# JuliaSmoothOptimizers/Krylov.jl

Hardware: NVIDIA H100
Metric: CG iterations/s (higher is better)
Workload: dtype f64

## Files before the change

krylov.jl_b200/csrc/blas1.cu:

```cuda
#include <mutex>
#include <set>
#include <utility>

#include "kb_internal.h"

#include <chrono>

namespace kb {

void ensure_dyn_smem(const void* func, int bytes) {
  static std::mutex mu;
  static std::set<std::pair<const void*, int>> done;
  int dev = 0;
  KB_CUDA(cudaGetDevice(&dev));
  std::lock_guard<std::mutex> lk(mu);
  if (done.count({func, dev})) return;
  KB_CUDA(cudaFuncSetAttribute(func, cudaFuncAttributeMaxDynamicSharedMemorySize, bytes));
  done.insert({func, dev});
}

double now_seconds() {
  using namespace std::chrono;
  return duration_cast<duration<double>>(steady_clock::now().time_since_epoch()).count();
}
// ... 265 lines not shown
  const long long code = (long long)s;
  user_exit = (code % 1024) > 0;
  overtimed = (code / 1024) > 0;
}

void dist_check_alive(Ctx& c) {
  if (!c.dcomm) return;
  int err = 0;
  KB_CUDA(cudaMemcpyAsync(&err, &c.dcomm->error, sizeof(int), cudaMemcpyDeviceToHost, c.stream));
  c.sync();
  if (err) throw std::runtime_error("cross-GPU reduction timed out: a peer rank stopped participating; the communicator of this "
                                    "workspace is dead (free the workspace on every rank and create it again)");
}

template <class T>
__global__ void __launch_bounds__(kBlock) cg_prologue_kernel(int n, const T* __restrict__ b, T* __restrict__ x, T* __restrict__ r,
                                                             T* __restrict__ p, T* part, unsigned* ticket, T* out, DistComm* dc) {
  __shared__ T sm[32];
  T acc = T(0);
  const int stride = gridDim.x * blockDim.x;
  for (int i = blockIdx.x * blockDim.x + threadIdx.x; i < n; i += stride) {
    const T v = b[i];
    x[i] = T(0); r[i] = v; p[i] = v;
    acc += v * v;
  }
  T mine[1] = {block_sum(acc, sm)}, tot[1];
  if (grid_sum_last<T, 1>(mine, part, ticket, sm, tot) && threadIdx.x == 0) out[0] = dist_reduce(dc, tot[0]);
}
template <class T> T k_cg_prologue(Ctx& c, int n, const T* b, T* x, T* r, T* p) {
  const int grid = n > 0 ? stream_grid(n, 4, 4) : 1;
  cg_prologue_kernel<T><<<grid, kBlock, 0, c.stream>>>(n, b, x, r, p, (T*)c.partials, c.tickets, slot_ptr<T>(c, 0), c.dcomm);
  KB_CUDA(cudaGetLastError());
  c.launches++;
  return read_slot<T>(c, 0);
}

#define INST(T)                                                                        \
  template T k_dot<T>(Ctx&, int, const T*, const T*);                                  \
  template T k_cg_prologue<T>(Ctx&, int, const T*, T*, T*, T*);                        \
  template T k_nrm2<T>(Ctx&, int, const T*);                                           \
  template void k_dot2<T>(Ctx&, int, const T*, const T*, const T*, const T*, T*, T*);  \
  template void k_dot_dev<T>(Ctx&, int, const T*, const T*, int);                      \
  template void k_axpy<T>(Ctx&, int, T, const T*, T*);                                 \
  template void k_axpby<T>(Ctx&, int, T, const T*, T, T*);                             \
  template void k_scal<T>(Ctx&, int, T, T*);                                           \
  template void k_copy<T>(Ctx&, int, T*, const T*);                                    \
  template void k_scalcopy<T>(Ctx&, int, T*, T, const T*);                             \
  template void k_divcopy<T>(Ctx&, int, T*, const T*, T);                              \
  template void k_fill<T>(Ctx&, int, T*, T);                                           \
  template void k_diagmul<T>(Ctx&, int, T*, const T*, const T*, bool);                 \
  template void k_blockdiag_mul<T>(Ctx&, int, int, const T*, const T*, T*);            \
  template void k_blockdiag_invert<T>(Ctx&, int, int, const T*, T*, int*);
INST(double)
INST(float)
// ... 4 lines not shown
```

krylov.jl_b200/csrc/cg_fused.cu:

```cuda
#include "solver_common.h"
#include "spmv_tiles.cuh"

namespace kb {

constexpr int kHist = 64;

template <class T>
struct CgState {
  T gamma, pAp, alpha, beta, pNorm2, rNorm, eps_tol, pad0;
  int iter, itmax, done, linesearch;
  int solved, tired, zero_curvature, inconsistent;
  int npc, not_spd, comm_error, pad2;
  T hist[kHist];
};

static_assert(sizeof(CgState<double>) % 8 == 0 && sizeof(CgState<float>) % 8 == 0, "CgState is copied as 8-byte words");

template <class T>
struct CgPeers {
  HaloMap halo;
  const T* r[kMaxRanks];
  const T* p_old[kMaxRanks];
  const T* mdiag;
  const T* r_halo;
  const T* p_halo_old;
  PushPlan<T> push_p;
};

template <class T>
// ... 335 lines not shown

template <class T>
__device__ __forceinline__ void cg_stage_halo(HaloMap halo, const CgPeerTab<T>* tab, T* r, T* p_old, int pb, int G, int tid, int nthreads) {
  const int nh = halo.nhalo, nloc = halo.nloc;
  const int per = (nh + G - 1) / G;
  const int h0 = (int)blockIdx.x * per, h1 = min(nh, h0 + per);
  for (int h = h0 + tid; h < h1; h += nthreads) {
    const int rk = __ldg(&halo.src_rank[h]), off = __ldg(&halo.src_off[h]);
    const T rv = ld_sys(tab->r[rk] + off);
    const T pv = ld_sys(tab->p[pb][rk] + off);
    __stcg(&r[nloc + h], rv);
    __stcg(&p_old[nloc + h], pv);
  }
}

template <class T, int MODE, class PhaseA>
__device__ __forceinline__ int cg_persist_iterations(int n, const CgPersistArgs<T>& a, CgState<T>* st, T* part, GridBar* gb,
                                                     DistComm* dc, T* sm, unsigned* sflag, CgScal<T>& sc, PhaseA phase_a) {
  const int G = gridDim.x, tid = threadIdx.x, lane = tid & 31;
  int passes = 0;
  for (int k = 0; k < a.max_iters; k++) {
    const int iter = sc.iter;
    const T beta = sc.beta, alpha_prev = sc.alpha;
    T* p_old = (iter & 1) ? a.P1 : a.P0;
    T* p_new = (iter & 1) ? a.P0 : a.P1;
    const bool timing = a.timed && blockIdx.x == 0 && tid == 0;
    unsigned long long t0 = 0, t1 = 0;
    if (timing) t0 = globaltimer_ns();
    const T dacc = phase_a(k, iter, beta, alpha_prev, p_old, p_new);
    passes = k + 1;
    bool ok = grid_reduce_barrier<T>(gb, dacc, part, sm, sflag, st, &sc, [&](T tot) {
      if (MODE == kDist) {
        tot = (T)dist_allreduce_sum_warp<T>(dc, (double)tot);
        if (*(volatile int*)&dc->error) { if (lane == 0) { st->comm_error = 1; st->done = 1; } return; }
      }
// ... 14 lines not shown
    }
    ok = grid_reduce_barrier<T>(gb, acc, part, sm, sflag, st, &sc, [&](T tot) {
      if (MODE == kDist) {
        tot = (T)dist_allreduce_sum_warp<T>(dc, (double)tot);
        if (*(volatile int*)&dc->error) { if (lane == 0) { st->comm_error = 1; st->done = 1; } return; }
      }
      if (lane == 0) {
        cg_k2_finalize(st, tot);
        if (MODE == kDist) gb->halo_ready = 0u;
      }
    });
    if (timing) {
      const unsigned long long t2 = globaltimer_ns();
      gb->ns_a += t1 - t0; gb->ns_b += t2 - t1; gb->timed_iters += 1;
    }
    if (!ok || sc.done) break;
  }
  return passes;
}

template <class T, int MODE, int MINB>
__global__ void __launch_bounds__(kTileThreads, MINB) cg_persist(Csr<T> A, CgPersistArgs<T> a, CgState<T>* st, T* part,
                                                                GridBar* gb, DistComm* dc) {
  extern __shared__ __align__(128) unsigned char smem[];
  __shared__ T sm[32];
  __shared__ unsigned sflag[2];
  __shared__ CgScal<T> sc;
  volatile CgState<T>* vst = st;
  if (vst->done) { cg_report_to_host<T>(a, st); return; }
  if (threadIdx.x == 0) cg_load_scal<T>(st, &sc);
  TilePipe<T> P;
// ... 177 lines not shown
    std::vector<int> fl(nt), ord;
    KB_CUDA(cudaMemcpyAsync(fl.data(), ws.dist.tile_order, sizeof(int) * nt, cudaMemcpyDeviceToHost, c.stream));
    c.sync();
    ord.reserve(nt);
    for (int t = 0; t < nt; t++) if (!fl[t]) ord.push_back(t);
    ws.dist.tile_order_interior = (int)ord.size();
    for (int t = 0; t < nt; t++) if (fl[t]) ord.push_back((int)((unsigned)t | 0x80000000u));
    KB_CUDA(cudaMemcpyAsync(ws.dist.tile_order, ord.data(), sizeof(int) * nt, cudaMemcpyHostToDevice, c.stream));
    c.sync();
  }
  ws.dist.tile_order_for = (const void*)A.rowptr;
  ws.dist.tile_order_n = nt;
}

template <class T>
CgFusedPlan<T> cg_fused_plan(const Workspace<T>& ws, const LinOp<T>& A, const LinOp<T>& M, const SolveOpts& o) {
  CgFusedPlan<T> pl;
  const bool dist = ws.dist.world > 1;
  const bool jac = M.kind == LinOp<T>::DIAG && !o.ldiv, bjac = M.kind == LinOp<T>::BDIAG && !o.ldiv;
  if (!o.fused || A.kind != LinOp<T>::CSR || o.radius != 0 || !(M.is_identity() || jac || bjac) || (dist && !M.is_identity()))
    return pl;
  const Csr<T>& C = *A.csr;
  const int n = ws.n;
  pl.single_step = (o.callback != nullptr) || (o.timemax < 1e300) || o.verbose > 0;
  const char* exu = getenv("KB200_XUP");
  pl.xup = !pl.single_step && !(exu && atoi(exu) == 0);
  pl.persist = C.tma_ok && pl.xup && o.persist != 0;
  if (bjac && !pl.persist) return pl;
  pl.fused = true;
  pl.A = &C;
  pl.mdiag = jac ? M.diag : nullptr;
  pl.mblocks = bjac ? M.blocks : nullptr;
  pl.mbs = bjac ? M.bs : 0;
  pl.batch = pl.single_step ? 1 : (o.batch > 0 ? std::min(o.batch, kHist / 2) : 32);
  if (pl.persist) {
    if (bjac) pl.kp = cg_persist<T, kBlockJac, 2>;
    else if (C.ctas_per_sm >= 3) pl.kp = dist ? cg_persist<T, kDist, 3> : (jac ? cg_persist<T, kJacobi, 3> : cg_persist<T, kPlain, 3>);
    else pl.kp = dist ? cg_persist<T, kDist, 2> : (jac ? cg_persist<T, kJacobi, 2> : cg_persist<T, kPlain, 2>);
    ensure_dyn_smem((const void*)pl.kp, 220 * 1024);
    int occ = 0;
    KB_CUDA(cudaOccupancyMaxActiveBlocksPerMultiprocessor(&occ, pl.kp, kTileThreads, C.smem_bytes));
    if (occ < 1) throw std::runtime_error("cg_persist does not fit on an SM with the planned shared-memory ring");
    pl.pgrid = std::min(std::min(occ, C.ctas_per_sm) * sm_count(), std::max(1, C.ntiles));
    const CsrDict<T>* dict = A.dict;
    if (dict && dict->npairs > 0 && dict->n == n && !dist && !bjac) {
      const typename CgFusedPlan<T>::KdFn kd =
          C.ctas_per_sm >= 3 ? (jac ? cg_persist_dict<T, kJacobi, 3> : cg_persist_dict<T, kPlain, 3>)
                             : (jac ? cg_persist_dict<T, kJacobi, 2> : cg_persist_dict<T, kPlain, 2>);
      int occd = 0;
      KB_CUDA(cudaOccupancyMaxActiveBlocksPerMultiprocessor(&occd, kd, kTileThreads, 0));
      if (occd * sm_count() >= pl.pgrid) { pl.kd = kd; pl.dict = dict; }
    }
    return pl;
  }
  const bool xup = pl.xup;
  if (C.tma_ok) {
    if (dist) pl.k1 = xup ? cg_k1_tma<T, kDist, 3, true> : cg_k1_tma<T, kDist, 3, false>;
    else if (jac) pl.k1 = xup ? cg_k1_tma<T, kJacobi, 3, true> : cg_k1_tma<T, kJacobi, 3, false>;
    else if (C.ctas_per_sm >= 4) pl.k1 = xup ? cg_k1_tma<T, kPlain, 4, true> : cg_k1_tma<T, kPlain, 4, false>;
    else if (C.ctas_per_sm == 3) pl.k1 = xup ? cg_k1_tma<T, kPlain, 3, true> : cg_k1_tma<T, kPlain, 3, false>;
    else pl.k1 = xup ? cg_k1_tma<T, kPlain, 1, true> : cg_k1_tma<T, kPlain, 1, false>;
    ensure_dyn_smem((const void*)pl.k1, 220 * 1024);
    int occ = 0;
    KB_CUDA(cudaOccupancyMaxActiveBlocksPerMultiprocessor(&occ, pl.k1, kTileThreads, C.smem_bytes));
    if (occ < 1) throw std::runtime_error("cg_k1_tma does not fit on an SM with the planned shared-memory ring");
    pl.k1_grid = std::min(std::min(occ, C.ctas_per_sm) * sm_count(), std::max(1, C.ntiles));
    pl.k1_block = kTileThreads;
    pl.k1_smem = C.smem_bytes;
  } else {
    if (dist) pl.k1 = xup ? cg_k1_rows<T, kDist, true> : cg_k1_rows<T, kDist, false>;
    else if (jac) pl.k1 = xup ? cg_k1_rows<T, kJacobi, true> : cg_k1_rows<T, kJacobi, false>;
    else pl.k1 = xup ? cg_k1_rows<T, kPlain, true> : cg_k1_rows<T, kPlain, false>;
    pl.k1_grid = stream_grid(n, 1, 8);
    pl.k1_block = kBlock;
    pl.k1_smem = 0;
  }
  if (dist) pl.k2 = xup ? cg_k2<T, kDist, false> : cg_k2<T, kDist, true>;
  else if (jac) pl.k2 = xup ? cg_k2<T, kJacobi, false> : cg_k2<T, kJacobi, true>;
  else pl.k2 = xup ? cg_k2<T, kPlain, false> : cg_k2<T, kPlain, true>;
  pl.k2_grid = stream_grid(n, 4, 8);
  return pl;
}

template <class T>
CgFusedExit cg_fused_loop(Workspace<T>& ws, const CgFusedPlan<T>& pl, const SolveOpts& o, T gamma0, T eps_tol, int itmax,
                          double start_time) {
  Ctx& c = ws.ctx;
  const int n = ws.n;
  typedef CgState<T> St;
  const bool dist = ws.dist.world > 1;
  const Csr<T>& A = *pl.A;
  cg_fused_prepare<T>(ws);
  St* dst = (St*)ws.fused_state;
  St* hst = (St*)ws.fused_host;
  auto hslot = [&](int i) -> St* { return (St*)((char*)hst + (size_t)i * kOffGridBar); };

  St init;
  memset(&init, 0, sizeof(init));
  init.gamma = gamma0; init.pNorm2 = gamma0; init.beta = T(0); init.eps_tol = eps_tol;
  init.rNorm = sqrt(gamma0); init.itmax = itmax; init.linesearch = o.linesearch ? 1 : 0;
  *hslot(0) = init;
  KB_CUDA(cudaMemcpyAsync(dst, hslot(0), sizeof(St), cudaMemcpyHostToDevice, c.stream));
  KB_CUDA(cudaMemsetAsync((char*)ws.fused_state + kOffGridBar, 0, sizeof(GridBar), c.stream));

  const bool persist = pl.persist, single_step = pl.single_step;
  const int batch = pl.batch;
  T* P[2] = {ws.p, ws.p2};
  T* part = (T*)c.partials;
  CgPeers<T> peersP[2];
  memset(peersP, 0, sizeof(peersP));
  const T* md = pl.mdiag;
  peersP[0].mdiag = md; peersP[1].mdiag = md;
  PushPlan<T> push_r;
  memset(&push_r, 0, sizeof(push_r));
  if (dist) {
    for (int b = 0; b < 2; b++) {
      peersP[b].halo = ws.dist.halo;
      const bool wantB = (b == 1) != ws.dist.swapped;
      for (int k = 0; k < ws.dist.world; k++) {
        peersP[b].r[k] = ws.dist.r_peer[k];
        peersP[b].p_old[k] = wantB ? ws.dist.bufB_peer[k] : ws.dist.bufA_peer[k];
// ... 33 lines not shown
        for (int k = 0; k < ws.dist.world; k++) {
          htab->r[k] = ws.dist.r_peer[k];
          htab->p[b][k] = wantB ? ws.dist.bufB_peer[k] : ws.dist.bufA_peer[k];
        }
      }
      CgPeerTab<T>* dtab = (CgPeerTab<T>*)((char*)ws.fused_state + kOffPeerTab);
      KB_CUDA(cudaMemcpyAsync(dtab, htab, sizeof(*htab), cudaMemcpyHostToDevice, c.stream));
      pa.halo = ws.dist.halo;
      pa.tab = dtab;
      pa.tile_order = ws.dist.tile_order;
      pa.n_interior = ws.dist.tile_order_interior;
    }
  }

  cudaEvent_t* ev = ws.fused_ev;
  int enq = 0;
  constexpr int kTimedFirst = 8, kTimedCount = 32;
  std::vector<cudaEvent_t> tev;
  if (o.time_kernels) {
    tev.resize(3 * kTimedCount);
    for (auto& e : tev) KB_CUDA(cudaEventCreate(&e));
  }
  unsigned long long* hseq = (unsigned long long*)((char*)ws.fused_host + kOffHostSeq);
  unsigned long long expect[2] = {0, 0};
  auto wait_report = [&](int slot) {
    long spins = 0;
    while (__atomic_load_n(&hseq[slot], __ATOMIC_ACQUIRE) != expect[slot]) {
      if ((++spins & 1023) == 0) {
        const cudaError_t q = cudaStreamQuery(c.stream);
        if (q != cudaSuccess && q != cudaErrorNotReady) throw CudaError(std::string("persistent CG kernel failed: ") + cudaGetErrorString(q));
        if (q == cudaSuccess && __atomic_load_n(&hseq[slot], __ATOMIC_ACQUIRE) != expect[slot])
// ... 16 lines not shown
        CsrDict<T> Dcopy = *pl.dict;
        void* args[] = {(void*)&Dcopy, (void*)&pa, (void*)&dst, (void*)&partp, (void*)&gbar};
        KB_CUDA(cudaLaunchCooperativeKernel((const void*)pl.kd, dim3(pl.pgrid), dim3(kTileThreads), args, 0, c.stream));
      } else {
        void* args[] = {(void*)&Acopy, (void*)&pa, (void*)&dst, (void*)&partp, (void*)&gbar, (void*)&dcm};
        KB_CUDA(cudaLaunchCooperativeKernel((const void*)pl.kp, dim3(pl.pgrid), dim3(kTileThreads), args, A.smem_bytes, c.stream));
      }
      c.launches += 1;
      enq += batch;
      return;
    }
    for (int b = 0; b < batch; b++, enq++) {
      T* p_old = P[enq & 1];
      T* p_new = P[(enq + 1) & 1];
      const CgPeers<T>& pe = peersP[enq & 1];
      const int ti = enq - kTimedFirst;
      const bool timed = o.time_kernels && ti >= 0 && ti < kTimedCount;
      if (timed) KB_CUDA(cudaEventRecord(tev[3 * ti], c.stream));
      DistComm* dcm = dist ? c.dcomm : nullptr;
      pl.k1<<<pl.k1_grid, pl.k1_block, pl.k1_smem, c.stream>>>(A, ws.r, p_old, p_new, ws.Ap, dst, part, c.tickets + 2, dcm, pe, ws.x);
      if (timed) KB_CUDA(cudaEventRecord(tev[3 * ti + 1], c.stream));
      pl.k2<<<pl.k2_grid, kBlock, 0, c.stream>>>(n, ws.x, ws.r, p_new, ws.Ap, dst, part, c.tickets + 3, dcm, md, push_r);
      if (timed) KB_CUDA(cudaEventRecord(tev[3 * ti + 2], c.stream));
      c.launches += 2;
    }
    KB_CUDA(cudaGetLastError());
    KB_CUDA(cudaMemcpyAsync(hslot(slot), dst, sizeof(St), cudaMemcpyDeviceToHost, c.stream));
    KB_CUDA(cudaEventRecord(ev[slot], c.stream));
  };

  int cur = 0, seen = 0;
  St last;
  bool user_exit = false, overtimed = false;
  enqueue(0);
  for (;;) {
    if (!single_step) enqueue(cur ^ 1);
    if (persist) wait_report(cur);
    else KB_CUDA(cudaEventSynchronize(ev[cur]));
    last = *hslot(cur);
    for (int k = seen + 1; k <= last.iter; k++) {
      if (o.history) ws.stats.residuals.push_back((double)last.hist[k % kHist]);
    }
    seen = last.iter;
    if (last.done) break;
    if (single_step) {
      if (o.verbose > 0 && (last.iter % o.verbose == 0))
        fprintf(stdout, "%5d  %7.1e  %8.1e  %8.1e\n", last.iter, (double)last.rNorm, (double)last.pAp, (double)last.alpha);
      if (o.callback) {
        ws.stats.niter = last.iter;
        user_exit = o.callback(&ws, o.callback_user) != 0;
      }
      overtimed = (now_seconds() - start_time) > o.timemax;
      agree_exit(ws, o, user_exit, overtimed);
      if (user_exit || overtimed) break;
      enqueue(cur);
    } else {
      cur ^= 1;
    }
  }
  c.sync();
  if (o.time_kernels && persist) {
    GridBar hb;
    KB_CUDA(cudaMemcpy(&hb, gbar, sizeof(hb), cudaMemcpyDeviceToHost));
    ws.timed_pairs = (int)hb.timed_iters;
    ws.k1_ms = hb.timed_iters ? 1e-6 * (double)hb.ns_a / hb.timed_iters : 0;
    ws.k2_ms = hb.timed_iters ? 1e-6 * (double)hb.ns_b / hb.timed_iters : 0;
    for (auto& e : tev) cudaEventDestroy(e);
  } else if (o.time_kernels) {
    const int pairs = std::min(kTimedCount, std::max(0, std::min(enq, last.iter) - kTimedFirst));
    double s1 = 0, s2 = 0;
    for (int i = 0; i < pairs; i++) {
      float a = 0, b = 0;
      cudaEventElapsedTime(&a, tev[3 * i], tev[3 * i + 1]);
      cudaEventElapsedTime(&b, tev[3 * i + 1], tev[3 * i + 2]);
      s1 += a; s2 += b;
    }
    ws.timed_pairs = pairs;
    ws.k1_ms = pairs ? s1 / pairs : 0;
    ws.k2_ms = pairs ? s2 / pairs : 0;
    for (auto& e : tev) cudaEventDestroy(e);
  }
  if (last.comm_error) throw std::runtime_error("cross-GPU all-reduce timed out: a peer rank is not participating");
  if (last.not_spd) throw std::runtime_error("The linear operator `A` or the preconditioner `M` is not symmetric positive definite.");

  const int iter = last.iter;
  const bool k1_exit = last.zero_curvature || last.npc;
  T* pcur = k1_exit ? P[(iter + 1) & 1] : P[iter & 1];
  if (pcur != ws.p) { T* tmp = ws.p; ws.p = ws.p2; ws.p2 = tmp; ws.dist.swapped = !ws.dist.swapped; }
  if (pl.xup && !k1_exit && iter > 0) k_axpy<T>(c, n, last.alpha, ws.p, ws.x);
  if (last.npc) {
    if (iter == 0) k_copy<T>(c, n, ws.x, ws.p);
    k_copy<T>(c, n, ws.npc_dir, ws.p);
    ws.stats.npcCount = 1;
    ws.stats.indefinite = true;
  }
  return CgFusedExit{iter, last.solved != 0, last.tired != 0, last.zero_curvature != 0, last.inconsistent != 0, user_exit, overtimed};
}

#define INST(T)                                                                                              \
  template CgFusedPlan<T> cg_fused_plan<T>(const Workspace<T>&, const LinOp<T>&, const LinOp<T>&, const SolveOpts&); \
  template void fused_block_alloc<T>(Workspace<T>&);                                                         \
  template void cg_fused_prepare<T>(Workspace<T>&);                                                          \
  template void cg_dist_push_r<T>(Workspace<T>&);                                                            \
  template CgFusedExit cg_fused_loop<T>(Workspace<T>&, const CgFusedPlan<T>&, const SolveOpts&, T, T, int, double);
INST(double)
INST(float)
#undef INST

}
```

krylov.jl_b200/csrc/kb_internal.h:

```cpp
#pragma once
#include <cuda_runtime.h>
#include <cstddef>
#include <cstdint>
#include <string>
#include <vector>

#include "common.cuh"
#include "dist.cuh"

namespace kb {

struct Ctx {
  int device = 0;
  cudaStream_t stream = nullptr;
  bool own_stream = false;
  void* partials = nullptr;
  unsigned* tickets = nullptr;
  void* dscal = nullptr;
  void* hscal = nullptr;
  long long launches = 0;
  DistComm* dcomm = nullptr;
  DistExchange* dex = nullptr;

  void init(int dev);
  void destroy();
  void sync() { KB_CUDA(cudaStreamSynchronize(stream)); }
};

template <class T> T* dev_alloc(size_t n);
void dev_free(void* p);

template <class T> T    k_dot(Ctx& c, int n, const T* x, const T* y);
template <class T> T    k_nrm2(Ctx& c, int n, const T* x);
template <class T> T    k_cg_prologue(Ctx& c, int n, const T* b, T* x, T* r, T* p);
template <class T> void k_dot2(Ctx& c, int n, const T* a, const T* b, const T* u, const T* v, T* r1, T* r2);
template <class T> void k_dot_dev(Ctx& c, int n, const T* x, const T* y, int slot);
template <class T> void k_axpy(Ctx& c, int n, T s, const T* x, T* y);
template <class T> void k_axpby(Ctx& c, int n, T s, const T* x, T t, T* y);
template <class T> void k_scal(Ctx& c, int n, T s, T* x);
template <class T> void k_copy(Ctx& c, int n, T* y, const T* x);
template <class T> void k_scalcopy(Ctx& c, int n, T* y, T s, const T* x);
template <class T> void k_divcopy(Ctx& c, int n, T* y, const T* x, T s);
template <class T> void k_fill(Ctx& c, int n, T* x, T v);
template <class T> void k_diagmul(Ctx& c, int n, T* y, const T* d, const T* x, bool ldiv);
template <class T> void k_blockdiag_mul(Ctx& c, int n, int bs, const T* blocks, const T* x, T* y);
template <class T> void k_blockdiag_invert(Ctx& c, int n, int bs, const T* blocks, T* inv, int* singular);
double k_dist_sum(Ctx& c, double v);
void dist_agree_on_exit(Ctx& c, bool& user_exit, bool& overtimed);
void dist_check_alive(Ctx& c);
// ... 225 lines not shown
  T *d1 = nullptr, *d2 = nullptr;
  T *Ar = nullptr, *Mr = nullptr;
  std::vector<T*> V;
  std::vector<T*> Z;
  std::vector<T> c, sgiv, zg, R;
  std::vector<T> err_vec;
  int memory = 20, window = 5;
  int inner_iter = 0;
  const T* mdiag_fused = nullptr;
  double k1_ms = 0, k2_ms = 0;
  int timed_pairs = 0;
  void* fused_state = nullptr;
  void* fused_host = nullptr;
  cudaEvent_t fused_ev[2] = {nullptr, nullptr};
  unsigned long long fused_seq = 0;
  T* bbuf = nullptr;
  T* cbuf = nullptr;
  struct Dist {
    int rank = 0, world = 1;
    HaloMap halo{0, 0, nullptr, nullptr};
    void* mailbox = nullptr;
    T* bufA_peer[kMaxRanks] = {};
    T* bufB_peer[kMaxRanks] = {};
    T* r_peer[kMaxRanks] = {};
    std::vector<void*> opened;
    bool swapped = false;
    T* halo_buf = nullptr;
    T* halo_buf_peer[kMaxRanks] = {};
    int nhalo_peer[kMaxRanks] = {};
    void* dummy[3] = {nullptr, nullptr, nullptr};
// ... 37 lines not shown
template <class T> void craig_solve(Workspace<T>& ws, const LinOp<T>& A, const LinOp<T>& At, const T* b, const LinOp<T>& M,
                                    const LinOp<T>& N, const SolveOpts& o);
template <class T> void craigmr_solve(Workspace<T>& ws, const LinOp<T>& A, const LinOp<T>& At, const T* b, const LinOp<T>& M,
                                      const LinOp<T>& N, const SolveOpts& o);
template <class T> void lnlq_solve(Workspace<T>& ws, const LinOp<T>& A, const LinOp<T>& At, const T* b, const LinOp<T>& M,
                                   const LinOp<T>& N, const SolveOpts& o);
template <class T> void cgne_solve(Workspace<T>& ws, const LinOp<T>& A, const LinOp<T>& At, const T* b, const LinOp<T>& N,
                                   const SolveOpts& o);
template <class T> void crmr_solve(Workspace<T>& ws, const LinOp<T>& A, const LinOp<T>& At, const T* b, const LinOp<T>& N,
                                   const SolveOpts& o);
template <class T> void cgls_solve(Workspace<T>& ws, const LinOp<T>& A, const LinOp<T>& At, const T* b, const LinOp<T>& M,
                                   const SolveOpts& o);
template <class T> void crls_solve(Workspace<T>& ws, const LinOp<T>& A, const LinOp<T>& At, const T* b, const LinOp<T>& M,
                                   const SolveOpts& o);

template <class T> struct CgState;
template <class T> struct CgPeers;
template <class T> struct CgPersistArgs;
struct GridBar;
template <class T>
struct CgFusedPlan {
  typedef void (*K1Fn)(Csr<T>, const T*, const T*, T*, T*, CgState<T>*, T*, unsigned*, DistComm*, CgPeers<T>, T*);
  typedef void (*K2Fn)(int, T*, T*, const T*, const T*, CgState<T>*, T*, unsigned*, DistComm*, const T*, PushPlan<T>);
  typedef void (*KpFn)(Csr<T>, CgPersistArgs<T>, CgState<T>*, T*, GridBar*, DistComm*);
  typedef void (*KdFn)(CsrDict<T>, CgPersistArgs<T>, CgState<T>*, T*, GridBar*);
  bool fused = false;
  bool persist = false;
  bool single_step = false;
  bool xup = false;
  int batch = 1;
  const Csr<T>* A = nullptr;
  const T* mdiag = nullptr;
  const T* mblocks = nullptr;
  int mbs = 0;
  K1Fn k1 = nullptr;
  K2Fn k2 = nullptr;
  int k1_grid = 0, k1_block = 0, k2_grid = 0;
  size_t k1_smem = 0;
  KpFn kp = nullptr;
  KdFn kd = nullptr;
  const CsrDict<T>* dict = nullptr;
  int pgrid = 0;
};
struct CgFusedExit { int iter; bool solved, tired, zero_curvature, inconsistent, user_exit, overtimed; };
template <class T> CgFusedPlan<T> cg_fused_plan(const Workspace<T>& ws, const LinOp<T>& A, const LinOp<T>& M, const SolveOpts& o);
template <class T> CgFusedExit cg_fused_loop(Workspace<T>& ws, const CgFusedPlan<T>& plan, const SolveOpts& o, T gamma0, T eps_tol,
                                             int itmax, double start_time);
template <class T> void cg_dist_push_r(Workspace<T>& ws);
template <class T> void cg_fused_prepare(Workspace<T>& ws);
template <class T> void fused_block_alloc(Workspace<T>& ws);
constexpr size_t kFusedBlockBytes = 4096;

template <class T> void bicgstab_fused_iteration(Workspace<T>& ws, const Csr<T>& A, const T* cvec, bool first, T rho_in, T* alpha,
                                                 T* omega, T* next_rho, T* rNorm);
template <class T> void minres_fused_lanczos(Workspace<T>& ws, const Csr<T>& A, int iter, T lambda, T beta, T oldbeta, T cs, T sn,
                                             T deltabar, T eps_rot, T* w, T* alpha, T* beta2);
template <class T> T minres_fused_update(Workspace<T>& ws, T* w, T gamma, T phi);
template <class T> void gmres_fused_arnoldi(Workspace<T>& ws, const Csr<T>& A, int k, T* h_out, T* Hbis, const T* xin = nullptr);
template <class T> void fused_multi_axpy(Workspace<T>& ws, T* xr, int k, const T* y, T* const* vecs);
template <class T> void fused_orth_chain(Workspace<T>& ws, const Csr<T>& A, const T* xin, T* q, const T* const* vecs, int cnt, T* h_out, T* Hbis);
template <class T> void trunc_fused_direction(Workspace<T>& ws, T* pp, int cnt, T* const* pvecs, const T* coefs, const T* z, T h0, T step);
template <class T> T cgs_fused_sigma(Workspace<T>& ws, const Csr<T>& A, const T* cvec);
// ... 63 lines not shown
```

krylov.jl_b200/csrc/solvers.cu:

```cuda
#include <algorithm>
#include <cmath>
#include <cstring>
#include <limits>

#include "solver_common.h"

namespace kb {

template <class T> Workspace<T>* ws_create(SolverKind kind, int m, int n, int memory, int window, int device) {
  const double t0 = now_seconds();
  const SolverInfo* info = solver_info(kind);
  if (m != n && !(info && info->rect)) throw std::runtime_error("System must be square");
  Workspace<T>* ws = new Workspace<T>();
  try {
    ws->kind = kind; ws->m = m; ws->n = n;
    ws->ctx.init(device);
    fused_block_alloc<T>(*ws);
    auto A = [&]() { return dev_alloc<T>((size_t)n); };
    ws->x = A();
    switch (kind) {
      case S_CG: ws->r = A(); ws->p = A(); ws->Ap = A(); cg_fused_prepare<T>(*ws); break;
      case S_BICGSTAB: ws->r = A(); ws->p = A(); ws->v = A(); ws->s = A(); ws->qd = A(); break;
      case S_MINRES:
        ws->r1 = A(); ws->r2 = A(); ws->w1 = A(); ws->w2 = A(); ws->y = A();
// ... 124 lines not shown
  const int n = ws.n;
  const T radius = (T)o.radius;
  const bool linesearch = o.linesearch, history = o.history, ldiv = o.ldiv;
  if (linesearch && radius > 0) throw std::runtime_error("`linesearch` set to `true` but trust-region radius > 0");
  if (ws.warm_start && linesearch) throw std::runtime_error("warm_start and linesearch cannot be used together");
  if (o.verbose > 0) printf("CG: system of %d equations in %d variables\n", n, n);
  const bool MisI = M.is_identity();
  allocate_if(!MisI, ws, ws.z);
  allocate_if(linesearch || radius > 0, ws, ws.npc_dir);
  T *dx = ws.dx, *x = ws.x, *r = ws.r, *Ap = ws.Ap;
  Stats& stats = ws.stats;
  const bool warm_start = ws.warm_start;
  stats.reset();
  T* z = MisI ? r : ws.z;

  T gamma;
  if (!warm_start && MisI && ws.dist.npush == 0) {
    gamma = k_cg_prologue<T>(c, n, b, x, r, ws.p);
  } else {
    k_fill<T>(c, n, x, T(0));
    if (warm_start) {
      op_apply(c, A, dx, r);
      k_axpby<T>(c, n, T(1), b, T(-1), r);
    } else {
      k_copy<T>(c, n, r, b);
    }
    cg_dist_push_r<T>(ws);
    if (!MisI) op_apply(c, M, r, z, ldiv);
    k_copy<T>(c, n, ws.p, z);
    gamma = k_dot<T>(c, n, r, z);
  }
  if (!(gamma >= 0)) throw std::runtime_error("The linear operator `A` or the preconditioner `M` is not symmetric positive definite.");
  T rNorm = std::sqrt(gamma);
  if (history) stats.residuals.push_back(rNorm);
  if (gamma == 0) { run.finish(0, true, false, "x is a zero-residual solution"); return; }
  int iter = 0;
  int itmax = default_itmax(ws, o.itmax);
  T pAp = 0, pNorm2 = gamma;
  const T eps_tol = tol_of<T>(o.atol) + tol_of<T>(o.rtol) * rNorm;
  if (o.verbose > 0) printf("%5s  %7s  %8s  %8s  %8s  %5s\n", "k", "‖r‖", "pAp", "α", "σ", "timer");
  if (kdisplay(iter, o.verbose)) printf("%5d  %7.1e", iter, (double)rNorm);
  bool solved = rNorm <= eps_tol, tired = iter >= itmax;
  bool inconsistent = false, on_boundary = false, zero_curvature = false, user_exit = false, overtimed = false;
  std::string status = "unknown";

  const CgFusedPlan<T> plan = (solved || tired) ? CgFusedPlan<T>() : cg_fused_plan<T>(ws, A, M, o);
  if (plan.fused) {
    const CgFusedExit e = cg_fused_loop<T>(ws, plan, o, gamma, eps_tol, itmax, run.start);
    iter = e.iter;
    solved = e.solved; tired = e.tired; zero_curvature = e.zero_curvature; inconsistent = e.inconsistent;
    user_exit = e.user_exit; overtimed = e.overtimed;
  } else {
    T* p = ws.p;
    while (!(solved || tired || zero_curvature || user_exit || overtimed)) {
      op_apply(c, A, p, Ap);
      pAp = k_dot<T>(c, n, p, Ap);
      if ((pAp <= eps_of<T>() * pNorm2) && (radius == 0)) {
        if (std::fabs(pAp) <= eps_of<T>() * pNorm2) { zero_curvature = true; inconsistent = !linesearch; }
        if (linesearch) {
          if (iter == 0) k_copy<T>(c, n, x, p);
          k_copy<T>(c, n, ws.npc_dir, p);
          stats.npcCount = 1; stats.indefinite = true; solved = true;
        }
// ... 564 lines not shown
```

Before: 3742.

## Seed CG state on device and run persistent solve without host round-trips

The CG prologue kernel now writes gamma, rNorm and eps_tol plus the early-exit flags straight into the device CgState, so the host no longer has to read gamma back before the fused loop starts. The persistent kernel can now run all iterations in one batch when history is off, and it applies the final x update inside the kernel instead of through a separate axpy launch. Occupancy queries are cached per workspace. Together these remove host synchronisations and kernel launches per solve. In exchange the early-exit and history logic becomes more complex, and not-SPD errors are detected lazily.

Result: no change. 3745, median of 6 (+0.1%).

```diff
diff --git a/krylov.jl_b200/csrc/blas1.cu b/krylov.jl_b200/csrc/blas1.cu
--- a/krylov.jl_b200/csrc/blas1.cu
+++ b/krylov.jl_b200/csrc/blas1.cu
@@ -303,8 +303,23 @@
 }
 
 template <class T>
+__device__ __forceinline__ void cg_state_seed(CgState<T>* st, T gamma, T atol, T rtol) {
+  st->gamma = gamma;
+  st->pNorm2 = gamma;
+  if (!(gamma >= T(0))) { st->not_spd = 1; st->done = 1; return; }
+  const T rNorm = sqrt_rn(gamma);
+  st->rNorm = rNorm;
+  st->rNorm0 = rNorm;
+  if (gamma == T(0)) { st->done = 1; return; }
+  const T eps_tol = add_rn(atol, mul_rn(rtol, rNorm));
+  st->eps_tol = eps_tol;
+  if (rNorm <= eps_tol) { st->solved = 1; st->done = 1; }
+}
+
+template <class T>
 __global__ void __launch_bounds__(kBlock) cg_prologue_kernel(int n, const T* __restrict__ b, T* __restrict__ x, T* __restrict__ r,
-                                                             T* __restrict__ p, T* part, unsigned* ticket, T* out, DistComm* dc) {
+                                                             T* __restrict__ p, T* part, unsigned* ticket, T* out, DistComm* dc,
+                                                             CgState<T>* st, T atol, T rtol) {
   __shared__ T sm[32];
   T acc = T(0);
   const int stride = gridDim.x * blockDim.x;
@@ -314,19 +329,31 @@
     acc += v * v;
   }
   T mine[1] = {block_sum(acc, sm)}, tot[1];
-  if (grid_sum_last<T, 1>(mine, part, ticket, sm, tot) && threadIdx.x == 0) out[0] = dist_reduce(dc, tot[0]);
+  if (grid_sum_last<T, 1>(mine, part, ticket, sm, tot) && threadIdx.x == 0) {
+    const T gamma = dist_reduce(dc, tot[0]);
+    if (st) cg_state_seed(st, gamma, atol, rtol);
+    else out[0] = gamma;
+  }
+}
+template <class T> static void cg_prologue_launch(Ctx& c, int n, const T* b, T* x, T* r, T* p, CgState<T>* st, T atol, T rtol) {
+  const int grid = n > 0 ? stream_grid(n, 4, 4) : 1;
+  cg_prologue_kernel<T><<<grid, kBlock, 0, c.stream>>>(n, b, x, r, p, (T*)c.partials, c.tickets, slot_ptr<T>(c, 0), c.dcomm,
+                                                       st, atol, rtol);
+  KB_CUDA(cudaGetLastError());
+  c.launches++;
 }
 template <class T> T k_cg_prologue(Ctx& c, int n, const T* b, T* x, T* r, T* p) {
-  const int grid = n > 0 ? stream_grid(n, 4, 4) : 1;
-  cg_prologue_kernel<T><<<grid, kBlock, 0, c.stream>>>(n, b, x, r, p, (T*)c.partials, c.tickets, slot_ptr<T>(c, 0), c.dcomm);
-  KB_CUDA(cudaGetLastError());
-  c.launches++;
+  cg_prologue_launch<T>(c, n, b, x, r, p, nullptr, T(0), T(0));
   return read_slot<T>(c, 0);
+}
+template <class T> void k_cg_prologue_seed(Ctx& c, int n, const T* b, T* x, T* r, T* p, CgState<T>* st, T atol, T rtol) {
+  cg_prologue_launch<T>(c, n, b, x, r, p, st, atol, rtol);
 }
 
 #define INST(T)                                                                        \
   template T k_dot<T>(Ctx&, int, const T*, const T*);                                  \
   template T k_cg_prologue<T>(Ctx&, int, const T*, T*, T*, T*);                        \
+  template void k_cg_prologue_seed<T>(Ctx&, int, const T*, T*, T*, T*, CgState<T>*, T, T); \
   template T k_nrm2<T>(Ctx&, int, const T*);                                           \
   template void k_dot2<T>(Ctx&, int, const T*, const T*, const T*, const T*, T*, T*);  \
   template void k_dot_dev<T>(Ctx&, int, const T*, const T*, int);                      \
diff --git a/krylov.jl_b200/csrc/cg_fused.cu b/krylov.jl_b200/csrc/cg_fused.cu
--- a/krylov.jl_b200/csrc/cg_fused.cu
+++ b/krylov.jl_b200/csrc/cg_fused.cu
@@ -2,17 +2,6 @@
 #include "spmv_tiles.cuh"
 
 namespace kb {
-
-constexpr int kHist = 64;
-
-template <class T>
-struct CgState {
-  T gamma, pAp, alpha, beta, pNorm2, rNorm, eps_tol, pad0;
-  int iter, itmax, done, linesearch;
-  int solved, tired, zero_curvature, inconsistent;
-  int npc, not_spd, comm_error, pad2;
-  T hist[kHist];
-};
 
 static_assert(sizeof(CgState<double>) % 8 == 0 && sizeof(CgState<float>) % 8 == 0, "CgState is copied as 8-byte words");
 
@@ -378,11 +367,18 @@
   }
 }
 
+template <class T>
+__device__ __forceinline__ void cg_persist_final_x(int n, T alpha, const T* p, T* x) {
+  const int stride = (int)(gridDim.x * blockDim.x);
+  for (int i = (int)(blockIdx.x * blockDim.x + threadIdx.x); i < n; i += stride) x[i] = add_rn(x[i], mul_rn(alpha, p[i]));
+}
+
 template <class T, int MODE, class PhaseA>
 __device__ __forceinline__ int cg_persist_iterations(int n, const CgPersistArgs<T>& a, CgState<T>* st, T* part, GridBar* gb,
                                                      DistComm* dc, T* sm, unsigned* sflag, CgScal<T>& sc, PhaseA phase_a) {
   const int G = gridDim.x, tid = threadIdx.x, lane = tid & 31;
   int passes = 0;
+  bool stopped_after_b = false;
   for (int k = 0; k < a.max_iters; k++) {
     const int iter = sc.iter;
     const T beta = sc.beta, alpha_prev = sc.alpha;
@@ -427,7 +423,15 @@
       const unsigned long long t2 = globaltimer_ns();
       gb->ns_a += t1 - t0; gb->ns_b += t2 - t1; gb->timed_iters += 1;
     }
-    if (!ok || sc.done) break;
+    if (!ok || sc.done) { stopped_after_b = ok; break; }
+  }
+  if (stopped_after_b) {
+    if (tid == 0) {
+      const volatile CgState<T>* v = st;
+      sflag[0] = !(v->not_spd || v->comm_error);
+    }
+    __syncthreads();
+    if (sflag[0]) cg_persist_final_x<T>(n, sc.alpha, (sc.iter & 1) ? a.P1 : a.P0, a.x);
   }
   return passes;
 }
@@ -635,7 +639,17 @@
 }
 
 template <class T>
-CgFusedPlan<T> cg_fused_plan(const Workspace<T>& ws, const LinOp<T>& A, const LinOp<T>& M, const SolveOpts& o) {
+static int cg_occupancy(Workspace<T>& ws, const void* kernel, size_t smem) {
+  for (const auto& e : ws.fused_occ)
+    if (e.first.first == kernel && e.first.second == smem) return e.second;
+  int occ = 0;
+  KB_CUDA(cudaOccupancyMaxActiveBlocksPerMultiprocessor(&occ, kernel, kTileThreads, smem));
+  ws.fused_occ.push_back({{kernel, smem}, occ});
+  return occ;
+}
+
+template <class T>
+CgFusedPlan<T> cg_fused_plan(Workspace<T>& ws, const LinOp<T>& A, const LinOp<T>& M, const SolveOpts& o) {
   CgFusedPlan<T> pl;
   const bool dist = ws.dist.world > 1;
   const bool jac = M.kind == LinOp<T>::DIAG && !o.ldiv, bjac = M.kind == LinOp<T>::BDIAG && !o.ldiv;
@@ -653,14 +667,13 @@
   pl.mdiag = jac ? M.diag : nullptr;
   pl.mblocks = bjac ? M.blocks : nullptr;
   pl.mbs = bjac ? M.bs : 0;
-  pl.batch = pl.single_step ? 1 : (o.batch > 0 ? std::min(o.batch, kHist / 2) : 32);
+  pl.batch = pl.single_step ? 1 : o.batch > 0 ? std::min(o.batch, kHist / 2) : (pl.persist && !o.history) ? 0 : 32;
   if (pl.persist) {
     if (bjac) pl.kp = cg_persist<T, kBlockJac, 2>;
     else if (C.ctas_per_sm >= 3) pl.kp = dist ? cg_persist<T, kDist, 3> : (jac ? cg_persist<T, kJacobi, 3> : cg_persist<T, kPlain, 3>);
     else pl.kp = dist ? cg_persist<T, kDist, 2> : (jac ? cg_persist<T, kJacobi, 2> : cg_persist<T, kPlain, 2>);
     ensure_dyn_smem((const void*)pl.kp, 220 * 1024);
-    int occ = 0;
-    KB_CUDA(cudaOccupancyMaxActiveBlocksPerMultiprocessor(&occ, pl.kp, kTileThreads, C.smem_bytes));
+    const int occ = cg_occupancy(ws, (const void*)pl.kp, C.smem_bytes);
     if (occ < 1) throw std::runtime_error("cg_persist does not fit on an SM with the planned shared-memory ring");
     pl.pgrid = std::min(std::min(occ, C.ctas_per_sm) * sm_count(), std::max(1, C.ntiles));
     const CsrDict<T>* dict = A.dict;
@@ -668,9 +681,7 @@
       const typename CgFusedPlan<T>::KdFn kd =
           C.ctas_per_sm >= 3 ? (jac ? cg_persist_dict<T, kJacobi, 3> : cg_persist_dict<T, kPlain, 3>)
                              : (jac ? cg_persist_dict<T, kJacobi, 2> : cg_persist_dict<T, kPlain, 2>);
-      int occd = 0;
-      KB_CUDA(cudaOccupancyMaxActiveBlocksPerMultiprocessor(&occd, kd, kTileThreads, 0));
-      if (occd * sm_count() >= pl.pgrid) { pl.kd = kd; pl.dict = dict; }
+      if (cg_occupancy(ws, (const void*)kd, 0) * sm_count() >= pl.pgrid) { pl.kd = kd; pl.dict = dict; }
     }
     return pl;
   }
@@ -682,8 +693,7 @@
     else if (C.ctas_per_sm == 3) pl.k1 = xup ? cg_k1_tma<T, kPlain, 3, true> : cg_k1_tma<T, kPlain, 3, false>;
     else pl.k1 = xup ? cg_k1_tma<T, kPlain, 1, true> : cg_k1_tma<T, kPlain, 1, false>;
     ensure_dyn_smem((const void*)pl.k1, 220 * 1024);
-    int occ = 0;
-    KB_CUDA(cudaOccupancyMaxActiveBlocksPerMultiprocessor(&occ, pl.k1, kTileThreads, C.smem_bytes));
+    const int occ = cg_occupancy(ws, (const void*)pl.k1, C.smem_bytes);
     if (occ < 1) throw std::runtime_error("cg_k1_tma does not fit on an SM with the planned shared-memory ring");
     pl.k1_grid = std::min(std::min(occ, C.ctas_per_sm) * sm_count(), std::max(1, C.ntiles));
     pl.k1_block = kTileThreads;
@@ -704,8 +714,8 @@
 }
 
 template <class T>
-CgFusedExit cg_fused_loop(Workspace<T>& ws, const CgFusedPlan<T>& pl, const SolveOpts& o, T gamma0, T eps_tol, int itmax,
-                          double start_time) {
+CgFusedExit cg_fused_loop(Workspace<T>& ws, const CgFusedPlan<T>& pl, const SolveOpts& o, const T* b_seed, T gamma0, T eps_tol,
+                          T atol, T rtol, int itmax, double start_time) {
   Ctx& c = ws.ctx;
   const int n = ws.n;
   typedef CgState<T> St;
@@ -723,9 +733,15 @@
   *hslot(0) = init;
   KB_CUDA(cudaMemcpyAsync(dst, hslot(0), sizeof(St), cudaMemcpyHostToDevice, c.stream));
   KB_CUDA(cudaMemsetAsync((char*)ws.fused_state + kOffGridBar, 0, sizeof(GridBar), c.stream));
+  const bool seeded = b_seed != nullptr;
+  if (seeded) k_cg_prologue_seed<T>(c, n, b_seed, ws.x, ws.r, ws.p, dst, atol, rtol);
 
   const bool persist = pl.persist, single_step = pl.single_step;
-  const int batch = pl.batch;
+  int batch = pl.batch;
+  if (batch == 0) {
+    const long long per_cta = std::max(1, (A.ntiles + pl.pgrid - 1) / std::max(1, pl.pgrid));
+    batch = (int)std::min<long long>(itmax, 0xFFFFFFFFLL / (per_cta + 1) - 1);
+  }
   T* P[2] = {ws.p, ws.p2};
   T* part = (T*)c.partials;
   CgPeers<T> peersP[2];
@@ -789,7 +805,7 @@
   }
 
   cudaEvent_t* ev = ws.fused_ev;
-  int enq = 0;
+  long long enq = 0;
   constexpr int kTimedFirst = 8, kTimedCount = 32;
   std::vector<cudaEvent_t> tev;
   if (o.time_kernels) {
@@ -836,7 +852,7 @@
       T* p_old = P[enq & 1];
       T* p_new = P[(enq + 1) & 1];
       const CgPeers<T>& pe = peersP[enq & 1];
-      const int ti = enq - kTimedFirst;
+      const long long ti = enq - kTimedFirst;
       const bool timed = o.time_kernels && ti >= 0 && ti < kTimedCount;
       if (timed) KB_CUDA(cudaEventRecord(tev[3 * ti], c.stream));
       DistComm* dcm = dist ? c.dcomm : nullptr;
@@ -853,13 +869,19 @@
 
   int cur = 0, seen = 0;
   St last;
-  bool user_exit = false, overtimed = false;
+  bool user_exit = false, overtimed = false, first_report = true;
   enqueue(0);
   for (;;) {
-    if (!single_step) enqueue(cur ^ 1);
+    const bool ahead = !single_step && enq < itmax;
+    if (ahead) enqueue(cur ^ 1);
     if (persist) wait_report(cur);
     else KB_CUDA(cudaEventSynchronize(ev[cur]));
     last = *hslot(cur);
+    if (seeded && first_report) {
+      if (last.iter == 0 && last.not_spd) dist_nan_guard(c, (double)last.gamma);
+      if (o.history && !last.not_spd) ws.stats.residuals.push_back((double)last.rNorm0);
+    }
+    first_report = false;
     for (int k = seen + 1; k <= last.iter; k++) {
       if (o.history) ws.stats.residuals.push_back((double)last.hist[k % kHist]);
     }
@@ -877,6 +899,7 @@
       if (user_exit || overtimed) break;
       enqueue(cur);
     } else {
+      if (!ahead) enqueue(cur ^ 1);
       cur ^= 1;
     }
   }
@@ -889,7 +912,7 @@
     ws.k2_ms = hb.timed_iters ? 1e-6 * (double)hb.ns_b / hb.timed_iters : 0;
     for (auto& e : tev) cudaEventDestroy(e);
   } else if (o.time_kernels) {
-    const int pairs = std::min(kTimedCount, std::max(0, std::min(enq, last.iter) - kTimedFirst));
+    const int pairs = (int)std::min<long long>(kTimedCount, std::max<long long>(0, std::min<long long>(enq, last.iter) - kTimedFirst));
     double s1 = 0, s2 = 0;
     for (int i = 0; i < pairs; i++) {
       float a = 0, b = 0;
@@ -909,22 +932,24 @@
   const bool k1_exit = last.zero_curvature || last.npc;
   T* pcur = k1_exit ? P[(iter + 1) & 1] : P[iter & 1];
   if (pcur != ws.p) { T* tmp = ws.p; ws.p = ws.p2; ws.p2 = tmp; ws.dist.swapped = !ws.dist.swapped; }
-  if (pl.xup && !k1_exit && iter > 0) k_axpy<T>(c, n, last.alpha, ws.p, ws.x);
+  if (pl.xup && !persist && !k1_exit && iter > 0) k_axpy<T>(c, n, last.alpha, ws.p, ws.x);
   if (last.npc) {
     if (iter == 0) k_copy<T>(c, n, ws.x, ws.p);
     k_copy<T>(c, n, ws.npc_dir, ws.p);
     ws.stats.npcCount = 1;
     ws.stats.indefinite = true;
   }
-  return CgFusedExit{iter, last.solved != 0, last.tired != 0, last.zero_curvature != 0, last.inconsistent != 0, user_exit, overtimed};
+  const bool zero_residual = seeded && iter == 0 && last.rNorm0 == T(0);
+  return CgFusedExit{iter, last.solved != 0, last.tired != 0, last.zero_curvature != 0, last.inconsistent != 0, user_exit, overtimed,
+                     zero_residual};
 }
 
 #define INST(T)                                                                                              \
-  template CgFusedPlan<T> cg_fused_plan<T>(const Workspace<T>&, const LinOp<T>&, const LinOp<T>&, const SolveOpts&); \
+  template CgFusedPlan<T> cg_fused_plan<T>(Workspace<T>&, const LinOp<T>&, const LinOp<T>&, const SolveOpts&);       \
   template void fused_block_alloc<T>(Workspace<T>&);                                                         \
   template void cg_fused_prepare<T>(Workspace<T>&);                                                          \
   template void cg_dist_push_r<T>(Workspace<T>&);                                                            \
-  template CgFusedExit cg_fused_loop<T>(Workspace<T>&, const CgFusedPlan<T>&, const SolveOpts&, T, T, int, double);
+  template CgFusedExit cg_fused_loop<T>(Workspace<T>&, const CgFusedPlan<T>&, const SolveOpts&, const T*, T, T, T, T, int, double);
 INST(double)
 INST(float)
 #undef INST
diff --git a/krylov.jl_b200/csrc/kb_internal.h b/krylov.jl_b200/csrc/kb_internal.h
--- a/krylov.jl_b200/csrc/kb_internal.h
+++ b/krylov.jl_b200/csrc/kb_internal.h
@@ -33,6 +33,8 @@
 template <class T> T    k_dot(Ctx& c, int n, const T* x, const T* y);
 template <class T> T    k_nrm2(Ctx& c, int n, const T* x);
 template <class T> T    k_cg_prologue(Ctx& c, int n, const T* b, T* x, T* r, T* p);
+template <class T> struct CgState;
+template <class T> void k_cg_prologue_seed(Ctx& c, int n, const T* b, T* x, T* r, T* p, CgState<T>* st, T atol, T rtol);
 template <class T> void k_dot2(Ctx& c, int n, const T* a, const T* b, const T* u, const T* v, T* r1, T* r2);
 template <class T> void k_dot_dev(Ctx& c, int n, const T* x, const T* y, int slot);
 template <class T> void k_axpy(Ctx& c, int n, T s, const T* x, T* y);
@@ -288,6 +290,7 @@
   void* fused_host = nullptr;
   cudaEvent_t fused_ev[2] = {nullptr, nullptr};
   unsigned long long fused_seq = 0;
+  std::vector<std::pair<std::pair<const void*, size_t>, int>> fused_occ;
   T* bbuf = nullptr;
   T* cbuf = nullptr;
   struct Dist {
@@ -355,7 +358,15 @@
 template <class T> void crls_solve(Workspace<T>& ws, const LinOp<T>& A, const LinOp<T>& At, const T* b, const LinOp<T>& M,
                                    const SolveOpts& o);
 
-template <class T> struct CgState;
+constexpr int kHist = 64;
+template <class T>
+struct CgState {
+  T gamma, pAp, alpha, beta, pNorm2, rNorm, eps_tol, rNorm0;
+  int iter, itmax, done, linesearch;
+  int solved, tired, zero_curvature, inconsistent;
+  int npc, not_spd, comm_error, pad2;
+  T hist[kHist];
+};
 template <class T> struct CgPeers;
 template <class T> struct CgPersistArgs;
 struct GridBar;
@@ -383,10 +394,10 @@
   const CsrDict<T>* dict = nullptr;
   int pgrid = 0;
 };
-struct CgFusedExit { int iter; bool solved, tired, zero_curvature, inconsistent, user_exit, overtimed; };
-template <class T> CgFusedPlan<T> cg_fused_plan(const Workspace<T>& ws, const LinOp<T>& A, const LinOp<T>& M, const SolveOpts& o);
-template <class T> CgFusedExit cg_fused_loop(Workspace<T>& ws, const CgFusedPlan<T>& plan, const SolveOpts& o, T gamma0, T eps_tol,
-                                             int itmax, double start_time);
+struct CgFusedExit { int iter; bool solved, tired, zero_curvature, inconsistent, user_exit, overtimed, zero_residual; };
+template <class T> CgFusedPlan<T> cg_fused_plan(Workspace<T>& ws, const LinOp<T>& A, const LinOp<T>& M, const SolveOpts& o);
+template <class T> CgFusedExit cg_fused_loop(Workspace<T>& ws, const CgFusedPlan<T>& plan, const SolveOpts& o, const T* b_seed,
+                                             T gamma0, T eps_tol, T atol, T rtol, int itmax, double start_time);
 template <class T> void cg_dist_push_r(Workspace<T>& ws);
 template <class T> void cg_fused_prepare(Workspace<T>& ws);
 template <class T> void fused_block_alloc(Workspace<T>& ws);
diff --git a/krylov.jl_b200/csrc/solvers.cu b/krylov.jl_b200/csrc/solvers.cu
--- a/krylov.jl_b200/csrc/solvers.cu
+++ b/krylov.jl_b200/csrc/solvers.cu
@@ -162,39 +162,47 @@
   stats.reset();
   T* z = MisI ? r : ws.z;
 
-  T gamma;
-  if (!warm_start && MisI && ws.dist.npush == 0) {
-    gamma = k_cg_prologue<T>(c, n, b, x, r, ws.p);
-  } else {
-    k_fill<T>(c, n, x, T(0));
-    if (warm_start) {
-      op_apply(c, A, dx, r);
-      k_axpby<T>(c, n, T(1), b, T(-1), r);
+  int iter = 0;
+  const int itmax = default_itmax(ws, o.itmax);
+  const T atol = tol_of<T>(o.atol), rtol = tol_of<T>(o.rtol);
+  const bool one_pass = !warm_start && MisI && ws.dist.npush == 0;
+  CgFusedPlan<T> plan = one_pass && itmax > 0 ? cg_fused_plan<T>(ws, A, M, o) : CgFusedPlan<T>();
+  const bool seeded = plan.persist;
+  T gamma = 0, rNorm = 0, eps_tol = 0;
+  if (!seeded) {
+    if (one_pass) {
+      gamma = k_cg_prologue<T>(c, n, b, x, r, ws.p);
     } else {
-      k_copy<T>(c, n, r, b);
-    }
-    cg_dist_push_r<T>(ws);
-    if (!MisI) op_apply(c, M, r, z, ldiv);
-    k_copy<T>(c, n, ws.p, z);
-    gamma = k_dot<T>(c, n, r, z);
-  }
-  if (!(gamma >= 0)) throw std::runtime_error("The linear operator `A` or the preconditioner `M` is not symmetric positive definite.");
-  T rNorm = std::sqrt(gamma);
-  if (history) stats.residuals.push_back(rNorm);
-  if (gamma == 0) { run.finish(0, true, false, "x is a zero-residual solution"); return; }
-  int iter = 0;
-  int itmax = default_itmax(ws, o.itmax);
+      k_fill<T>(c, n, x, T(0));
+      if (warm_start) {
+        op_apply(c, A, dx, r);
+        k_axpby<T>(c, n, T(1), b, T(-1), r);
+      } else {
+        k_copy<T>(c, n, r, b);
+      }
+      cg_dist_push_r<T>(ws);
+      if (!MisI) op_apply(c, M, r, z, ldiv);
+      k_copy<T>(c, n, ws.p, z);
+      gamma = k_dot<T>(c, n, r, z);
+    }
+    if (!(gamma >= 0)) throw std::runtime_error("The linear operator `A` or the preconditioner `M` is not symmetric positive definite.");
+    rNorm = std::sqrt(gamma);
+    if (history) stats.residuals.push_back(rNorm);
+    if (gamma == 0) { run.finish(0, true, false, "x is a zero-residual solution"); return; }
+    eps_tol = atol + rtol * rNorm;
+  }
   T pAp = 0, pNorm2 = gamma;
-  const T eps_tol = tol_of<T>(o.atol) + tol_of<T>(o.rtol) * rNorm;
   if (o.verbose > 0) printf("%5s  %7s  %8s  %8s  %8s  %5s\n", "k", "‖r‖", "pAp", "α", "σ", "timer");
   if (kdisplay(iter, o.verbose)) printf("%5d  %7.1e", iter, (double)rNorm);
-  bool solved = rNorm <= eps_tol, tired = iter >= itmax;
+  bool solved = !seeded && rNorm <= eps_tol, tired = iter >= itmax;
   bool inconsistent = false, on_boundary = false, zero_curvature = false, user_exit = false, overtimed = false;
   std::string status = "unknown";
 
-  const CgFusedPlan<T> plan = (solved || tired) ? CgFusedPlan<T>() : cg_fused_plan<T>(ws, A, M, o);
+  if (solved || tired) plan = CgFusedPlan<T>();
+  else if (!one_pass) plan = cg_fused_plan<T>(ws, A, M, o);
   if (plan.fused) {
-    const CgFusedExit e = cg_fused_loop<T>(ws, plan, o, gamma, eps_tol, itmax, run.start);
+    const CgFusedExit e = cg_fused_loop<T>(ws, plan, o, seeded ? b : nullptr, gamma, eps_tol, atol, rtol, itmax, run.start);
+    if (e.zero_residual) { run.finish(0, true, false, "x is a zero-residual solution"); return; }
     iter = e.iter;
     solved = e.solved; tired = e.tired; zero_curvature = e.zero_curvature; inconsistent = e.inconsistent;
     user_exit = e.user_exit; overtimed = e.overtimed;
diff --git a/profiles/trace_cg_step.py b/profiles/trace_cg_step.py
--- /dev/null
+++ b/profiles/trace_cg_step.py
@@ -0,0 +1,136 @@
+import argparse
+import json
+import os
+import subprocess
+import sys
+import tempfile
+
+ROOT = os.path.dirname(os.path.dirname(os.path.abspath(__file__)))
+
+CHILD = r'''
+import json, os, sys
+sys.path[:0] = [%(root)r, os.path.join(%(root)r, "krylov.jl_b200")]
+import numpy as np, torch
+import krylov_b200 as kb
+from krylov_b200.problems import div_grad_csr
+mode, steps, trace_dir = sys.argv[1], int(sys.argv[2]), sys.argv[3]
+N, ITERS = 215, 200
+dev = torch.device("cuda", 0)
+torch.cuda.set_device(0)
+rp, ci, va = div_grad_csr(N, xp=torch, device=dev)
+n = N ** 3
+b = torch.ones(n, dtype=torch.float64, device=dev)
+ws = kb.CgWorkspace(n, n, np.float64, device="cuda")
+ws.set_operator((rp, ci, va))
+kw = dict(atol=0.0, rtol=0.0, itmax=ITERS)
+for _ in range(3):
+    ws.solve(None, b, **kw)
+stream = torch.cuda.ExternalStream(kb.lib().krylov_b200_stream(ws._h), device=dev)
+lib = os.path.basename(os.environ.get("KB200_LIB", "tree"))
+if mode == "time":
+    e0, e1 = torch.cuda.Event(enable_timing=True), torch.cuda.Event(enable_timing=True)
+    l0 = ws.launches
+    torch.cuda.synchronize(); e0.record(stream)
+    for _ in range(steps):
+        ws.solve(None, b, **kw)
+    e1.record(stream); torch.cuda.synchronize()
+    ms = e0.elapsed_time(e1) / steps
+    launches = (ws.launches - l0) / steps
+    ws.solve(None, b, time_kernels=True, **kw)
+    a, bb, timed = ws.kernel_times
+    print(json.dumps(dict(kind="time", lib=lib, steps=steps, ms_step=ms, phase_a_ms=a, phase_b_ms=bb, timed_iterations=timed,
+                          ms_phases=ITERS * (a + bb), gap_ms=ms - ITERS * (a + bb), launches_per_solve=launches,
+                          niter=ws.stats.niter)))
+else:
+    from torch.profiler import profile, ProfilerActivity
+    torch.cuda.synchronize()
+    with profile(activities=[ProfilerActivity.CPU, ProfilerActivity.CUDA]) as prof:
+        for _ in range(3):
+            ws.solve(None, b, **kw)
+        torch.cuda.synchronize()
+    path = os.path.join(trace_dir, "cg_step_%%s.pt.trace.json" %% lib.replace(".so", ""))
+    prof.export_chrome_trace(path)
+    ev = json.load(open(path))["traceEvents"]
+    dev_ev = sorted((e for e in ev if e.get("cat") in ("kernel", "gpu_memcpy", "gpu_memset") and "dur" in e),
+                    key=lambda e: e["ts"])
+    rows, split, solve, end = [], {}, -1, None
+    persist_seen = False
+    for e in dev_ev:
+        name = e["name"]
+        gap = 0.0 if end is None else max(0.0, e["ts"] - end)
+        if "cg_prologue" in name:
+            solve += 1
+            where = "between_solves"
+            persist_seen = False
+        elif "cg_persist" in name:
+            where = "after_prologue" if not persist_seen else "between_launches"
+            persist_seen = True
+        elif "ew_kernel" in name or "axpy" in name:
+            where = "before_axpy"
+            split["axpy"] = split.get("axpy", 0.0) + e["dur"]
+        elif persist_seen and e["cat"] in ("gpu_memcpy", "gpu_memset"):
+            where = "between_solves"        # the next solve's set-up, enqueued before its prologue
+        else:
+            where = "between_launches" if persist_seen else "after_prologue"
+        if end is not None and solve >= 0:
+            split[where] = split.get(where, 0.0) + gap
+        rows.append(dict(solve=solve, name=name[:80], cat=e["cat"], dur_us=round(e["dur"], 2), gap_before_us=round(gap, 2),
+                         where=where))
+        end = e["ts"] + e["dur"] if end is None else max(end, e["ts"] + e["dur"])
+    solves = max(1, solve + 1)
+    print(json.dumps(dict(kind="trace", lib=lib, solves=solves, events=rows,
+                          idle_us_per_solve={k: round(v / solves, 1) for k, v in split.items()},
+                          trace=os.path.basename(path))))
+'''
+
+
+def gpu_info():
+    q = subprocess.run(["nvidia-smi", "--query-gpu=name,power.limit,clocks.max.sm", "--format=csv,noheader"],
+                       capture_output=True, text=True).stdout.strip().splitlines()
+    return q[0] if q else "unknown"
+
+
+def child(lib, mode, steps, trace_dir):
+    env = dict(os.environ)
+    env.pop("KB200_LIB", None)
+    if lib:
+        env["KB200_LIB"] = os.path.abspath(lib)
+    r = subprocess.run([sys.executable, "-c", CHILD % dict(root=ROOT), mode, str(steps), trace_dir], env=env,
+                       capture_output=True, text=True, cwd=ROOT)
+    lines = [l for l in r.stdout.splitlines() if l.startswith("{")]
+    if r.returncode != 0 or not lines:
+        raise SystemExit(f"child {mode} failed ({lib or 'tree'}): {r.stderr[-3000:]}")
+    return json.loads(lines[-1])
+
+
+def main():
+    ap = argparse.ArgumentParser()
+    ap.add_argument("--lib", action="append", default=[], help="another library build to alternate with the tree's")
+    ap.add_argument("--rounds", type=int, default=3)
+    ap.add_argument("--steps", type=int, default=10)
+    ap.add_argument("--trace-dir", default=None, help="where the chrome traces go (default: a temporary directory)")
+    ap.add_argument("--out", default=None)
+    args = ap.parse_args()
+    libs = args.lib + [None]
+    out = [dict(kind="gpu", gpu=gpu_info())]
+    print(json.dumps(out[0]), flush=True)
+    with tempfile.TemporaryDirectory() as tmp:
+        tdir = args.trace_dir or tmp
+        os.makedirs(tdir, exist_ok=True)
+        for _ in range(args.rounds):
+            for lib in libs:
+                out.append(child(lib, "time", args.steps, tdir))
+                print(json.dumps(out[-1]), flush=True)
+        for lib in libs:
+            out.append(child(lib, "trace", 0, tdir))
+            t = out[-1]
+            print(json.dumps(dict(kind="trace", lib=t["lib"], idle_us_per_solve=t["idle_us_per_solve"])), flush=True)
+    out.append(dict(kind="gpu", gpu=gpu_info()))
+    if args.out:
+        with open(args.out, "a") as f:
+            for rec in out:
+                f.write(json.dumps(rec) + "\n")
+
+
+if __name__ == "__main__":
+    main()
```
